# DelftMercurians/Parallax

Hardware: AMD Instinct MI355X
Metric: env steps/sec (whole node), RoboCup 4096 envs/GPU, at 1/2/4/8 MI355X (higher is better)
Workload: dtype f32

## Files before the change

__graft_entry__.py:

```python
import os
import subprocess
import sys

ROOT = os.path.dirname(os.path.abspath(__file__))
CSRC = os.path.join(ROOT, "parallax_amd", "csrc")
HIP_SRC = os.path.join(CSRC, "cotix_step.hip")
HIP_KERNEL_SRC = os.path.join(CSRC, "cotix_step_kernel.hip")
HIP_LIB = os.path.join(ROOT, "parallax_amd", "_lib", "libcotix_amd.so")
HIPCC_FLAGS = ["-O3", "--offload-arch=gfx950", "-ffp-contract=off", "-fno-fast-math", "-std=c++17", "-fPIC"]


def _run(cmd, cwd=ROOT):
    print("+", " ".join(cmd), flush=True)
    subprocess.run(cmd, cwd=cwd, check=True)


def build_id(defines=(), extra=()):
    import hashlib
    h = hashlib.sha256()
    files = sorted(f for f in os.listdir(CSRC) if f.endswith((".h", ".hip")))
    for f in files:
        h.update(f.encode())
        h.update(open(os.path.join(CSRC, f), "rb").read())
    h.update(open(os.path.join(ROOT, "include", "cotix_amd.h"), "rb").read())
# ... 10 lines not shown
    os.makedirs(os.path.dirname(out), exist_ok=True)
    hipcc = os.environ.get("HIPCC", "/opt/rocm/bin/hipcc")
    objdir = os.path.join(ROOT, "parallax_amd", "_lib", "obj", os.path.basename(out).replace(".so", ""))
    os.makedirs(objdir, exist_ok=True)
    flags = [*HIPCC_FLAGS, *["-D" + d for d in defines], *extra]
    bid = build_id(defines, extra)
    jobs = [([hipcc, *flags, '-DCOTIX_BUILD_ID="%s"' % bid, "-c", HIP_SRC,
              "-o", os.path.join(objdir, "cotix_step.o")])]
    for ew in ews:
        jobs.append([hipcc, *flags, "-DCOTIX_EW=%d" % ew, "-c", HIP_KERNEL_SRC,
                     "-o", os.path.join(objdir, "cotix_step_kernel_ew%d.o" % ew)])
    stamps = {cmd[-1]: " ".join(cmd) + "\nbuild_id " + bid for cmd in jobs}
    procs = []
    for cmd in jobs:
        if not _stale(cmd[-1], stamps[cmd[-1]]):
            continue
        print("+", " ".join(cmd), flush=True)
        procs.append((cmd, subprocess.Popen(cmd, cwd=ROOT)))
    rcs = [p.wait() for _, p in procs]
    if any(rc != 0 for rc in rcs):
        raise RuntimeError("hipcc failed (%d of %d objects)" % (sum(rc != 0 for rc in rcs), len(rcs)))
    for cmd, _ in procs:
        with open(cmd[-1] + ".cmd", "w") as f:
            f.write(stamps[cmd[-1]])
    _run([hipcc, *flags, "-shared", *[j[-1] for j in jobs], "-o", out])


def build_checkers():
    _run(["make", "-s", "-C", os.path.join(ROOT, "oracle")])
    _run(["make", "-s", "-C", os.path.join(ROOT, "tests", "emu"), "build/libcotix_emu.so"])
    _run(["make", "-s", "-C", os.path.join(ROOT, "tests", "emu"), "-f", "gradp.mk", "build/libcotix_emu_gradp.so"])
    _run(["make", "-s", "-C", os.path.join(ROOT, "tests", "emu"), "-f", "evalgrad.mk",
          "build/libcotix_emu_evalgrad.so"])


def build():
    build_hip()
    build_checkers()
    sys.path.insert(0, ROOT)
    import parallax_amd
    print("built", HIP_LIB)


def smoke():
    import numpy as np
    import torch

    sys.path.insert(0, ROOT)
    sys.path.insert(0, os.path.join(ROOT, "oracle"))
    import parallax_amd as pa
    from cotix_oracle import geometry as G
    from cotix_oracle import physics as P
    from cotix_oracle import prng

    assert torch.cuda.is_available(), "smoke() needs a GPU"
    d0 = prng.gjk_initial_direction()

    env = pa.RoboCupEnv(batch=1, device="cuda:0", keys=pa.random.PRNGKey(0, "cuda:0")[None])
    env.world.step(3, 1e-2, env.stages)
    torch.cuda.synchronize()
    got = env.world.dyn[:, :, 0].cpu().numpy()
    bodies, key = P.robocup_bodies(), prng.PRNGKey(0)
    for _ in range(3):
        bodies, key = P.robocup_step(bodies, key, d0, G.ErrorFlag())
    want = np.array([b.dyn() for b in bodies], dtype=np.float32)
    assert np.array_equal(np.isnan(got), np.isnan(want)), (got, want)
# ... 17 lines not shown
```

parallax_amd/csrc/cotix_kernel.h:

```cpp
#pragma once
#include "../../include/cotix_amd.h"
#include "cotix_device.h"
#include "cotix_grad.h"

namespace cxk {

constexpr int MAXB = 16, MAXP = 32, MAXC = 256, MAXL = 128, MAXT = 13, MAXCAND = 16384;
constexpr int MAXHOT = 24576;
constexpr int WAVE = 64;

#ifdef COTIX_STATS
struct Stats {
  unsigned long long wave_steps, active_items, rounds, resolutions, f_items, b_items, draws, valid_draws, r1_left, lvl_env, lvl_wave, e1_slots;
  unsigned long long valid_cands, fit64;
  unsigned long long bp_cand, bp_guard_fail;
  unsigned long long epa_runs;
};
inline Stats g_stats{};
#define CXK_STAT(f, v) (cxk::g_stats.f += (unsigned long long)(v))
#else
#define CXK_STAT(f, v) ((void)0)
#endif
#if defined(COTIX_PHASE_PROF) && (defined(__HIP__) || defined(__HIPCC__))
static __device__ unsigned long long g_sub_cycles[8];
#define CXK_SUB_T0 const unsigned long long cxk_sub_t0 = clock64()
#define CXK_SUB_T1(k, lane)                                                                       \
  do {                                                                                            \
    const unsigned long long dt_ = clock64() - cxk_sub_t0;                                        \
    if ((lane) == __builtin_amdgcn_readfirstlane(lane)) atomicAdd(&cxk::g_sub_cycles[k], dt_); \
  } while (0)
#else
#define CXK_SUB_T0 ((void)0)
#define CXK_SUB_T1(k, lane) ((void)0)
#endif

#define CXK_INLINE_LAMBDA __attribute__((always_inline))

#ifdef COTIX_TOOLING
#define CXK_SKIP(a, bit) (((a).dbg_skip & (bit)) != 0)
#else
#define CXK_SKIP(a, bit) false
#endif

#define CXK_HDR_FIELDS(X)                                                                                          \
  X(uint16_t, nb) X(uint16_t, np) X(uint16_t, nc) X(uint16_t, nl) X(uint16_t, nt) X(uint16_t, G) X(uint16_t, W)   \
  X(uint16_t, ncand) X(float, d0x) X(float, d0y) X(uint16_t, o_par) X(uint16_t, o_rcp) X(uint16_t, o_pbody)     \
  X(uint16_t, o_pkind) X(uint16_t, o_pn) X(uint16_t, o_pgoff) X(uint16_t, o_pwoff) X(uint16_t, o_cpa)           \
  X(uint16_t, o_cpb) X(uint16_t, o_cfn) X(uint16_t, o_ci) X(uint16_t, o_cj) X(uint16_t, o_cbeg) X(uint16_t, o_ccnt) \
  X(uint16_t, o_tn1) X(uint16_t, o_tn2) X(uint16_t, o_cand) X(uint16_t, o_cdesc) X(uint16_t, o_cmask)          \
  X(uint16_t, o_cbody) X(uint16_t, nmw) X(uint16_t, poly) X(uint16_t, rcp_all) X(uint16_t, fnset)               \
  X(uint16_t, nhot) X(uint16_t, nvt) X(uint16_t, o_vit) X(uint32_t, rcp_mask) X(uint16_t, maxv)                 \
  X(uint16_t, pminv) X(uint16_t, prng) X(uint16_t, gjk_steps) X(uint16_t, epa_cap) X(uint16_t, epa_cp)          \
  X(uint16_t, epa_body) X(float, baum) X(float, baum_dt) X(float, pc) X(uint16_t, epar)
struct SceneHdr {
// ... 1737 lines not shown
  bool any = false;
  for (int q = 0; q < sc.nmw; ++q) any |= (t.tb[sc.o_cmask + l * sc.nmw + q] & t.w(c.L.vm + q, e)) != 0u;
  return any;
}
template <int EW, bool L1 = false>
CX_DEV uint32_t m_draw(const Ctx& c, Tile<EW> t, uint32_t sw, int q, int kso, bool& pass, int kl1 = 0, int ko1 = 0) {
  using namespace cx;
  const SceneHdr& sc = c.sh;
  pass = false;
  const int base = (int)(sw & 4095u), end = (int)((sw >> 12) & 8191u), id = (int)(sw >> 25);
  const int e = id % EW, idx = base + q;
  if (idx >= end) return 0xFFFFFFFFu;
  const uint32_t cd = t.tb[sc.o_cand + idx];
  const int i1 = cd & 511u, i2 = (cd >> 9) & 511u, cid = (cd >> 18) & 511u, ty = cd >> 27;
  const float cpx = t.f(c.L.con + 4 * cid + 2, e), cpy = t.f(c.L.con + 4 * cid + 3, e);
  int ko = i2;
  if constexpr (L1) {
    ko += ty > 0 ? ko1 : 0;
    for (int p = 1; p + 1 < c.nt; ++p) ko += p < ty ? t.ti(sc.o_tn2 + p) : 0;
  }
  const key2 sk = L1 ? key2{t.w(kl1 + 2 * ko, e), t.w(kl1 + 2 * ko + 1, e)}
                     : key2{t.w(kso + 2 + 2 * ty, e), t.w(kso + 3 + 2 * ty, e)};
  const bool part = sc.prng != 0;
  const bool valid = !(isn(cpx) || isn(cpy));
  const key2 k2 = L1 ? sk : split_at_l(sk, (uint32_t)t.ti(sc.o_tn2 + ty), (uint32_t)i2, part);
  const key2 k = split_at_l(k2, (uint32_t)t.ti(sc.o_tn1 + ty), (uint32_t)i1, part);
  pass = bernoulli_l(split_at_l(k, 2u, 0u, part), sc.pc, part) & valid;
  CXK_STAT(draws, 1);
  CXK_STAT(valid_draws, valid ? 1 : 0);
  return cd;
}
struct MItem {
  int cb = 0, ce = 0, cell = 0, pos = 0, e = 0;
};
template <int EW>
CX_DEV MItem m_item(const Ctx& c, Tile<EW> t, int id) {
  const SceneHdr& sc = c.sh;
  MItem it;
  if (id < c.nl * EW) {
    const int l = id / EW;
    it.e = id % EW;
    it.cb = t.ti(sc.o_cbeg + l);
    it.ce = it.cb + t.ti(sc.o_ccnt + l);
    it.cell = c.L.m + t.ti(sc.o_ci + l) * c.nb + t.ti(sc.o_cj + l);
  }
  return it;
}
struct MConst {
  MItem it[2];
  uint32_t cm[2][2] = {{0u, 0u}, {0u, 0u}};
};
template <int EW>
CX_DEV void mc_fetch(const Ctx& c, Tile<EW> t, int lane, MConst& m) {
  const SceneHdr& sc = c.sh;
#pragma unroll
  for (int s = 0; s < 2; ++s) {
    const int id = lane + s * WAVE;
    if (s == 1 && c.nl * EW <= WAVE) continue;
    m.it[s] = m_item<EW>(c, t, id);
    if (id < c.nl * EW)
      for (int q = 0; q < 2 && q < sc.nmw; ++q) m.cm[s][q] = t.tb[sc.o_cmask + (id / EW) * sc.nmw + q];
  }
}
template <int EW>
CX_DEV bool m0_active_c(const KArgs& a, const Ctx& c, Tile<EW> t, int env0, int id, const uint32_t* cm) {
  const SceneHdr& sc = c.sh;
  if (sc.nmw > 2) return m0_active<EW>(a, c, t, env0, id);
  if (id >= c.nl * EW) return false;
  const int e = id % EW;
  if (env0 + e >= a.B) return false;
  bool any = false;
  for (int q = 0; q < 2 && q < sc.nmw; ++q) any |= (cm[q] & t.w(c.L.vm + q, e)) != 0u;
  return any;
}
template <int EW>
CX_DEV bool m_settle(Tile<EW> t, MItem& it, bool drew, uint64_t bits, uint32_t wcd, int G) {
  if (!drew) return true;
  if (bits != 0ull) {
    t.w(it.cell, it.e) = wcd;
    return false;
  }
  it.pos += G;
  return it.cb + it.pos < it.ce;
}
template <int EW, bool L1 = false>
CX_DEV void ph_M_fused(const KArgs& a, const Ctx& c, Tile<EW> t, int env0, int lane, int kso, const MConst& mc,
                       int kl1 = 0, int ko1 = 0) {
  const bool two = c.nl * EW > WAVE;
  MItem it0 = mc.it[0], it1 = mc.it[1];
  const bool f0 = m0_active_c<EW>(a, c, t, env0, lane, mc.cm[0]);
  const bool f1 = two && m0_active_c<EW>(a, c, t, env0, lane + WAVE, mc.cm[1]);
  uint64_t pend0 = ballot(f0), pend1 = two ? ballot(f1) : 0ull;
#ifdef COTIX_STATS
  {
    uint64_t nv = 0;
    for (int s = 0; s < 2; ++s) {
      const MItem& it = s ? it1 : it0;
      if (!(s ? f1 : f0)) continue;
      for (int idx = it.cb; idx < it.ce; ++idx) {
        const int cid = (t.tb[c.sh.o_cand + idx] >> 18) & 511u;
        if (!(cx::isn(t.f(c.L.con + 4 * cid + 2, it.e)) || cx::isn(t.f(c.L.con + 4 * cid + 3, it.e)))) ++nv;
      }
    }
    static uint64_t wsum = 0;
    if (lane == 0) wsum = 0;
    wsum += nv;
    if (lane == WAVE - 1) {
      CXK_STAT(valid_cands, wsum);
      CXK_STAT(fit64, wsum <= 64 ? 1 : 0);
      CXK_STAT(wave_steps, 1);
      CXK_STAT(active_items, popc64(pend0) + popc64(pend1));
    }
  }
#endif
  for (int round = 0; (pend0 | pend1) != 0ull; ++round) {
#ifdef COTIX_STATS
    if (lane == 0) {
      CXK_STAT(rounds, 1);
      if (round == 1) CXK_STAT(r1_left, popc64(pend0) + popc64(pend1));
    }
#endif
    const int n0 = popc64(pend0), n = n0 + popc64(pend1);
    const int ns = n < COTIX_SCAN_RANKS ? n : COTIX_SCAN_RANKS, G = lanes_per_item(ns);
    const bool m0 = ((pend0 >> lane) & 1ull) != 0ull, m1 = ((pend1 >> lane) & 1ull) != 0ull;
    const int r0 = popc64(pend0 & lanes_below(lane)), r1 = n0 + popc64(pend1 & lanes_below(lane));
    const bool d0 = m0 && r0 < ns, d1 = m1 && r1 < ns;
    if (d0) t.ws[WS_FLAG + r0] = (uint32_t)(it0.cb + it0.pos) | ((uint32_t)it0.ce << 12) | ((uint32_t)lane << 25);
    if (d1)
      t.ws[WS_FLAG + r1] =
          (uint32_t)(it1.cb + it1.pos) | ((uint32_t)it1.ce << 12) | ((uint32_t)(lane + WAVE) << 25);
    lockstep();
    const int slot = rank_of_lane(lane, G), q = lane - slot * G;
    bool pass = false;
    uint32_t cd = 0xFFFFFFFFu;
    if (slot < ns) cd = m_draw<EW, L1>(c, t, t.ws[WS_FLAG + slot], q, kso, pass, kl1, ko1);
    const uint64_t pm = ballot(pass);
    const uint64_t gm = G == WAVE ? ~0ull : ((1ull << G) - 1ull);
    const uint64_t b0 = d0 ? (pm >> (r0 * G)) & gm : 0ull;
    const uint32_t w0 = bpermute(b0 != 0ull ? r0 * G + __builtin_ctzll(b0) : lane, cd);
    const bool k0 = m0 && m_settle<EW>(t, it0, d0, b0, w0, G);
    pend0 = ballot(k0);
    if (two) {
      const uint64_t b1 = d1 ? (pm >> (r1 * G)) & gm : 0ull;
      const uint32_t w1 = bpermute(b1 != 0ull ? r1 * G + __builtin_ctzll(b1) : lane, cd);
      const bool k1 = m1 && m_settle<EW>(t, it1, d1, b1, w1, G);
      pend1 = ballot(k1);
    }
  }
}

CX_DEV cx::Params load_par(const uint32_t* tb, int o) {
  return cx::Params{__uint_as_float(tb[o]), __uint_as_float(tb[o + 1]), __uint_as_float(tb[o + 2]),
                    __uint_as_float(tb[o + 3])};
}
template <int EW>
CX_DEV cx::Params body_par(const Ctx& c, Tile<EW> t, int i, int e) {
  if (c.sh.epar == 0) return load_par(t.tb, c.sh.o_par + 4 * i);
  const int o = c.L.geo + (int)c.sh.epar - 1 + 4 * i;
  return cx::Params{t.f(o, e), t.f(o + 1, e), t.f(o + 2, e), t.f(o + 3, e)};
}
CX_DEV cx::Rcp load_rcp(const uint32_t* tb, int o) {
  return cx::Rcp{__uint_as_float(tb[o]), __uint_as_float(tb[o + 1])};
}

CX_HD int tape_stage(const Ctx& c) { return c.L.rec - 5 * c.nb; }
template <int EW, bool RCP>
CX_DEV void e0_item(const Ctx& c, Tile<EW> t, int e, int i, int j, int cid, bool stage = false, uint32_t* tp = nullptr) {
  using namespace cx;
  const SceneHdr& sc = c.sh;
  const Lay& L = c.L;
  const int ro = L.rp + RP_W * i;
  const bool pair = !(j == i || j < 0 || j >= c.nb) && cid >= 0;
  const int jc = pair ? j : i, co = L.con + 4 * (pair ? cid : 0);
  const v2 cp = v2{t.f(co + 2, e), t.f(co + 3, e)};
  const int oi = L.dyn + 6 * i, oj = L.dyn + 6 * jc;
  const Dyn bi = Dyn{t.f(oi, e), t.f(oi + 1, e), 0.0f, 0.0f, 0.0f, 0.0f};
  const Dyn bj = Dyn{t.f(oj, e), t.f(oj + 1, e), 0.0f, 0.0f, 0.0f, 0.0f};
  const Params pj = body_par<EW>(c, t, jc, e);
  const Rcp qj = load_rcp(t.tb, sc.o_rcp + 2 * jc);
  const ResPre p = resolve_pre<RCP>(bi, body_par<EW>(c, t, i, e), load_rcp(t.tb, sc.o_rcp + 2 * i), bj, pj, qj,
                                    v2{t.f(co, e), t.f(co + 1, e)}, cp, baum_of(sc));
// ... 1398 lines not shown
    int e = w % EW, off = w / EW, g = env0 + e;
    if (g < a.B) a.grad_dyn[(size_t)off * a.B + g] = t.f(c.L.adj + off, e);
  }
}

enum : int { PH_LOAD, PH_SAVE, PH_A, PH_T, PH_B, PH_C0, PH_C0B, PH_C1, PH_C2, PH_C3, PH_D, PH_E, PH_RET, PH_STORE,
             PH_RESTORE, PH_G, PH_ADJ, PH_F, PH_K, PH_E1, PH_R, PH_TRACE, PH_BP0, PH_BP1, PH_F0, PH_F1, PH_F2, PH_F3,
             PH_TV0, PH_TV1, PH_TV2, PH_TV3, PH_J, PH_GE, PH_COUNT };
template <int EW, int FNSET, class R>
CX_DEV void transform_phases(const KArgs& a, const Ctx& c, Tile<EW> t, int env0, const R& run) {
  {
    run(PH_T, [&](int l) { ph_T<EW, FNSET>(a, c, t, env0, l); });
    if (FNSET != FNS_ANALYTIC && c.sh.nvt > 0) {
      uint64_t redo = 0ull;
      uint32_t runs = 0u;
      run(PH_TV1, [&](int l) {
        ph_TV0<EW>(a, c, t, env0, l);
        redo = tv_redo_mask<EW>(c, t, l);
        runs = tv_chunks<EW>(c, t, redo);
        ph_TV1<EW>(a, c, t, env0, l, redo, runs);
      });
      run(PH_TV2, [&](int l) { ph_TV2<EW>(a, c, t, env0, l, redo, runs); });
      run(PH_TV3, [&](int l) { ph_TV3<EW>(a, c, t, env0, l, redo, runs); });
      if ((FNSET & FNS_CONVEX) != 0 && c.sh.poly && (a.stages & COTIX_STAGE_BROADPHASE) && !CXK_SKIP(a, 2))
        run(PH_TV3, [&](int l) { ph_TV4<EW>(a, c, t, env0, l, redo, runs); });
#ifdef COTIX_EMU_POISON
      run(PH_TV3, [&](int l) {
        for (int q = l; q < 3 * c.sh.nvt * EW; q += WAVE) t.ws[c.W.vt + q] = 0x7FBADBADu;
      });
#endif
    }
  }
}
template <int EW, int FNSET, bool PRE, class R, bool AB = false, bool TAPE = false, bool L1 = false>
CX_DEV void collider_phases(const KArgs& a, const Ctx& c, Tile<EW> t, int env0, const R& run, int slot, int kso,
                            const MConst& mc, int step = 0, int kl1 = 0, int ko1 = 0) {
  if (!AB && !CXK_SKIP(a, 1)) transform_phases<EW, FNSET>(a, c, t, env0, run);
  if ((FNSET & FNS_CONVEX) != 0 && c.sh.poly && (a.stages & COTIX_STAGE_BROADPHASE) && !CXK_SKIP(a, 2)) {
    run(PH_BP0, [&](int l) { ph_BP0<EW>(a, c, t, env0, l); });
    const int n = (int)t.ws[c.W.bl_n];
    CXK_STAT(b_items, 0);
    const bool pairs = b_pairs<FNSET>() && t.ws[c.W.bl_mode] != 0u;
    const int per_round = pairs ? WAVE / 2 : WAVE;
    for (int r = 0; r * per_round < n; ++r)
      run(PH_B, [&](int l) { ph_BP2<EW, FNSET, TAPE>(a, c, t, env0, l, r, pairs, step); });
  } else if (!AB && !CXK_SKIP(a, 2)) {
    run(PH_B, [&](int l) { ph_B<EW, FNSET, TAPE>(a, c, t, env0, l, step); });
  }
  if ((FNSET & FNS_CONVEX) != 0 && c.sh.poly && !CXK_SKIP(a, 2)) {
    for (int ch = 0; ch * WAVE < c.nc * EW; ++ch) run(PH_F0, [&](int l) { ph_F0<EW>(c, t, l, ch); });
    const int n = (int)t.ws[c.W.cf_n];
    CXK_STAT(f_items, n);
    for (int b = 0; b < n; b += CFB) {
      run(PH_F1, [&](int l) { ph_F1<EW>(c, t, l, b); });
      int TC = 0, TE = 0;
      for (int i = 0; i < CFB; ++i) {
        TC += (int)t.ws[c.W.cf_c + i];
        TE += (int)t.ws[c.W.cf_s + i] - (int)t.ws[c.W.cf_c + i];
      }
      for (int r = 0; r * WAVE < TC; ++r) run(PH_F2, [&](int l) { ph_F2<EW, false>(c, t, l, b, r); });
      for (int r = 0; r * WAVE < TE; ++r) run(PH_F2, [&](int l) { ph_F2<EW, true>(c, t, l, b, r); });
      run(PH_F3, [&](int l) { ph_F3<EW>(c, t, l, b); });
    }
  }
  if (!CXK_SKIP(a, 4) && c.nl > 0 && scan_fused<EW>(c)) {
    run(PH_C1, [&](int l) { ph_M_fused<EW, L1>(a, c, t, env0, l, kso, mc, kl1, ko1); });
  } else if (!CXK_SKIP(a, 4) && c.nl > 0) {
    for (int ch = 0; ch * WAVE < c.nl * EW; ++ch) {
      run(PH_C0, [&](int l) { ph_C0<EW>(a, c, t, env0, l, ch); });
      run(PH_C0B, [&](int l) { ph_C0b<EW>(c, t, l, ch); });
    }
    CXK_STAT(wave_steps, 1);
    CXK_STAT(active_items, t.ws[WS_N]);
    for (int par = 0; t.ws[WS_N] != 0u; par ^= 1) {
      CXK_STAT(rounds, 1);
      run(PH_C1, [&](int l) { ph_C1<EW>(a, c, t, l, par, kso); });
      run(PH_C2, [&](int l) { ph_C2<EW>(c, t, l, par); });
      run(PH_C3, [&](int l) { ph_C3<EW>(c, t, l, par); });
    }
  }
  if (!CXK_SKIP(a, 8)) run(PH_D, [&](int l) { ph_D<EW, PRE, TAPE>(a, c, t, env0, l, kso, step); });
}

template <int EW, bool ROLL, bool EVAL = false>
CX_DEV void ph_load_fwd(const KArgs& a, const Ctx& c, Tile<EW> t, int env0, int l) {
  const float r0 = (ROLL && l < EW && env0 + l < a.B) ? a.ret[env0 + l] : 0.0f;
  ph_load<EW, EVAL>(a, c, t, env0, l);
  if (ROLL) {
    for (int e = l; e < EW; e += WAVE) {
      t.f(c.L.ret, e) = 0.0f;
      t.f(c.L.nres, e) = r0;
    }
    stage_ret_terms<EW>(a, c, t, l);
  }
}
struct NoKeyHelp {
  static constexpr bool on = false;
  int kwalt = 0;
  CX_MF void bar() const {}
// ... 42 lines not shown
template <int EW>
CX_HD int help_region_words(const Ctx& c) { return (c.L.S * EW + c.W.words + EW - 1) / EW * EW; }
template <int EW>
CX_HD size_t help_lds_bytes(const SceneHdr& s, int wpb) {
  const Ctx c = make_ctx<EW>(s);
  return 4 * ((size_t)s.nhot + (size_t)wpb * (help_region_words<EW>(c) + KWIN * c.L.kww * EW));
}

constexpr int KL1R = 8;
static_assert(KWIN % KL1R == 0, "a key window is whole ring halves (key_l1_next's barrier order)");
template <class H, class = void>
struct help_l1 {
  static constexpr bool value = false;
};
template <class H>
struct help_l1<H, decltype((void)H::l1)> {
  static constexpr bool value = H::l1;
};
template <class H>
CX_MF int help_l1o(const H& h) {
  if constexpr (help_l1<H>::value)
    return h.l1o;
  else
    return 0;
}
CX_HD int key_l1_keys(const SceneHdr& s, const uint32_t* tb) {
  int n = 0;
  for (int q = 0; q < s.nt; ++q) n += (int)tb[s.o_tn2 + q];
  return n;
}
template <int EW>
CX_HD int key_l1_ring_words(int nk1) { return 2 * KL1R * 2 * nk1 * EW; }
template <int EW>
CX_HD size_t help_l1_lds_bytes(const SceneHdr& s, int wpb, int nk1) {
  return help_lds_bytes<EW>(s, wpb) + 4 * (size_t)wpb * key_l1_ring_words<EW>(nk1);
}
CX_HD int key_l1_barriers(const KArgs& a) {
  return keys_on(a) && a.n_steps > 0 ? (a.n_steps + KL1R - 1) / KL1R : 0;
}
template <int EW>
struct KeyL1 {
  KeyHelper<EW> kh;
  int l1o = 0;
  int nk1 = 0;
  int s0 = 0;
  int q = 0;
};
template <int EW>
CX_DEV void key_l1_fill(const Ctx& c, Tile<EW> tr, Tile<EW> tk, int l1o, int nk1, int s0, int n, int lane) {
  using namespace cx;
  const SceneHdr& sc = c.sh;
  const bool part = sc.prng != 0;
#ifdef COTIX_EMU_POISON
  for (int w = lane; w < KL1R * 2 * nk1 * EW; w += WAVE)
    tr.u[(l1o + (s0 % (2 * KL1R)) * 2 * nk1) * EW + w] = 0x7FBADBADu;
  lockstep();
#endif
  for (int s = s0; s < s0 + n; ++s) {
    const int ko = c.L.kw + (s % KWIN) * c.L.kww, ro = l1o + (s % (2 * KL1R)) * 2 * nk1;
    for (int w = lane; w < nk1 * EW; w += WAVE) {
      const int e = w % EW;
      int j = w / EW, ty = 0, off = 0;
      for (int p = 0; p + 1 < c.nt; ++p) {
        const int np = tk.ti(sc.o_tn2 + p);
        if (ty == p && j >= np) {
          j -= np;
          off += np;
          ty = p + 1;
        }
      }
      const uint32_t N = (uint32_t)tk.ti(sc.o_tn2 + ty);
      const key2 sk = key2{tk.w(ko + 2 + 2 * ty, e), tk.w(ko + 3 + 2 * ty, e)};
      if (part) {
        const key2 k = split_at_l(sk, N, (uint32_t)j, true);
        tr.w(ro + 2 * (off + j), e) = k.a;
        tr.w(ro + 2 * (off + j) + 1, e) = k.b;
      } else {
        const key2 r = threefry(sk, (uint32_t)j, N + (uint32_t)j);
        tr.w(ro + 2 * off + j, e) = r.a;
        tr.w(ro + 2 * off + (int)N + j, e) = r.b;
      }
    }
  }
}
template <int EW, class R>
CX_DEV void key_l1_next(const KArgs& a, const Ctx& c, KeyL1<EW>& h, const R& run) {
  KeyHelper<EW>& kh = h.kh;
  if (h.q++ == 0) {
    const int n0 = a.n_steps < KWIN ? a.n_steps : KWIN;
    run(PH_K, [&](int l) {
      const int e = l >> 1, g = kh.env0 + e;
      if (l < 2 * EW && g < a.B) kh.k = cx::key2{a.keys[2 * (size_t)g], a.keys[2 * (size_t)g + 1]};
      k0_regs<EW>(a, c, kh.th, l, n0, kh.k, true);
    });
    run(PH_K, [&](int l) { ph_K1<EW>(c, kh.th, l, n0); });
  }
  if (h.s0 > 0 && h.s0 % KWIN == 0) key_helper_next<EW>(a, c, kh, run);
  const int w = h.s0 / KWIN, n = a.n_steps - h.s0 < KL1R ? a.n_steps - h.s0 : KL1R;
  const Tile<EW> tk = (w == 0 || (w & 1)) ? kh.th : kh.tm;
  run(PH_K, [&](int l) { key_l1_fill<EW>(c, kh.tm, tk, h.l1o, h.nk1, h.s0, n, l); });
  h.s0 += KL1R;
}

template <int EW, int FNSET, bool ROLL, bool EVAL = false, bool SDEFER = false, bool ESAVE = false, class R = void,
          class H = NoKeyHelp>
CX_DEV void run_wave(const KArgs& a, const Ctx& c, Tile<EW> t, int env0, const R& run, bool loaded = false,
                     const H& help = H{}) {
  static_assert(!(ROLL && EVAL), "the rollout has no judge");
  static_assert(!ESAVE || (EVAL && !ROLL && !SDEFER), "the saving eval is the eval program");
  static_assert(!(H::on && (ROLL || EVAL)), "the key helper runs the step program only");
  constexpr bool SAVE = ROLL || ESAVE;
  uint32_t fin0 = 0u;
  if (!loaded) run(PH_LOAD, [&](int l) { ph_load_fwd<EW, ROLL, EVAL>(a, c, t, env0, l); });
  const bool keys = keys_on(a);
  constexpr bool L1 = help_l1<H>::value;
  static_assert(!L1 || H::on, "the level-1 key ring is the key helper's");
  const int nk1 = L1 ? key_l1_keys(c.sh, t.tb) : 0, ko1 = L1 && c.nt > 0 ? t.ti(c.sh.o_tn2) : 0;
  if (EVAL && a.judge.on) {
    run(PH_J, [&](int l) {
      ph_JB<EW>(a, c, t, env0, l);
      if (ESAVE) ph_jrec<EW>(a, c, t, env0, l, 0, fin0);
    });
    run(PH_J, [&](int l) { ph_JS<EW>(c, t, l); });
  }

  const bool bconst = FNSET == FNS_ANALYTIC && c.nc * EW > ABQ * WAVE && c.nc * EW <= HQ * WAVE &&
                      (a.stages & COTIX_STAGE_COLLIDER) != 0 && !CXK_SKIP(a, 2) &&
                      a.n_steps >= COTIX_BCONST_MIN_STEPS;
  BConst bc;
  if (bconst) run(PH_B, [&](int l) { bc_fetch<EW>(c, t, l, bc); });
  MConst mc;
  if ((a.stages & COTIX_STAGE_COLLIDER) && c.nl > 0 && scan_fused<EW>(c))
    run(PH_C1, [&](int l) { mc_fetch<EW>(c, t, l, mc); });
  RetRegs rr;
  if (ROLL) run(PH_RET, [&](int l) { ret_fetch<EW>(c, t, l, rr); });
  const bool awin = ROLL && act_window<EW>(a, c);
  const bool apf = ROLL ? awin : act_prefetch<EW>(a, c);
  ActRegs an, ac;
  if (!ROLL && apf) run(PH_A, [&](int l) { act_fetch<EW>(a, c, env0, l, 0, an); });
  auto act_next = [&](int l, int step) {
    if (ROLL) {
      if (awin) {
        const int o = c.L.rst + 2 * (step % AWIN);
        ac.x = t.f(o, l % EW);
        ac.y = t.f(o + 1, l % EW);
      }
    } else {
      ac = an;
      if (apf && !a.action_held && step + 1 < a.n_steps) act_fetch<EW>(a, c, env0, l, step + 1, an);
    }
  };
  const bool staged = !bconst && FNSET == FNS_ANALYTIC && c.nc * EW <= ABQ * WAVE;
  const bool defer = restart_deferred(a) && (!staged || SDEFER);
  const bool rstore = a.dyn_reset != nullptr && a.reset_mode == 1 && !(EVAL && a.judge.on);
  for (int step = 0; step < a.n_steps; ++step) {
    if (awin && step % AWIN == 0) run(PH_K, [&](int l) { act_window_fill<EW>(a, c, t, env0, l, step); });
    if (SAVE) run(PH_SAVE, [&](int l) { ph_save<EW, FNSET == FNS_ANALYTIC>(a, c, t, env0, l, step); });
    const int slot = step % KWIN;
    if (H::on && keys && slot == 0 && step > 0) {
      help.bar();
    } else if (keys && slot == 0 && !(step == 0 && k_in_prologue(a))) {
      const int n = a.n_steps - step < KWIN ? a.n_steps - step : KWIN;
      if (n == 1) {
        run(PH_K, [&](int l) {
          const uint32_t k0 = l < EW ? t.w(c.L.key, l) : 0u, k1 = l < EW ? t.w(c.L.key + 1, l) : 0u;
          k_one_regs<EW>(a, c, t, l, k0, k1);
        });
      } else {
        run(PH_K, [&](int l) { ph_K0<EW>(a, c, t, l, n); });
        run(PH_K, [&](int l) { ph_K1<EW>(c, t, l, n); });
        if (a.stages & COTIX_STAGE_COLLIDER) run(PH_K, [&](int l) { ph_K2<EW>(c, t, l, n); });
      }
    }
    const int kso = c.L.kw + (H::on && ((step / KWIN) & 1) ? help.kwalt : 0) + slot * c.L.kww;
    const int kl1 = L1 ? help_l1o(help) + (step % (2 * KL1R)) * 2 * nk1 : 0;
    const bool l1bar = L1 && keys && step % KL1R == 0 && !(slot == 0 && step > 0);
    if (bconst) {
      run(PH_A, [&](int l) {
        act_next(l, step);
        ph_A<EW, true, EVAL, true>(a, c, t, env0, l, step, slot, apf, ac);
      });
      if (a.stages & COTIX_STAGE_COLLIDER) run(PH_B, [&](int l) { ph_B_const<EW>(a, c, t, env0, l, bc); });
      if (l1bar) help.bar();
      if (a.stages & COTIX_STAGE_COLLIDER)
        collider_phases<EW, FNSET, true, R, true, SAVE, L1>(a, c, t, env0, run, slot, kso, mc, step, kl1, ko1);
    } else if (FNSET == FNS_ANALYTIC && c.nc * EW <= ABQ * WAVE) {
      run.template staged<ABRegs>(
          PH_B, [&](int l, ABRegs& r) { ab_fetch<EW, SDEFER>(a, c, t, l, r); },
          [&](int l) {
            act_next(l, step);
            ph_A<EW, true, EVAL, SDEFER>(a, c, t, env0, l, step, slot, apf, ac);
          },
          [&](int l, const ABRegs& r) { ab_contacts<EW>(a, c, t, env0, l, r); });
      if (l1bar) help.bar();
      if (a.stages & COTIX_STAGE_COLLIDER) collider_phases<EW, FNSET, true, R, FNSET == FNS_ANALYTIC, SAVE, L1>(
          a, c, t, env0, run, slot, kso, mc, step, kl1, ko1);
    } else {
      run(PH_A, [&](int l) {
        act_next(l, step);
        ph_A<EW, true, EVAL, true>(a, c, t, env0, l, step, slot, apf, ac);
      });
      if (l1bar) help.bar();
      if (a.stages & COTIX_STAGE_COLLIDER)
        collider_phases<EW, FNSET, true, R, false, SAVE, L1>(a, c, t, env0, run, slot, kso, mc, step, kl1, ko1);
    }
    if (a.trace_chosen != nullptr || a.trace_cells != nullptr)
      run(PH_TRACE, [&](int l) { ph_trace<EW>(a, c, t, env0, l, step); });
    if (!CXK_SKIP(a, 32)) {
      if (SAVE && FNSET == FNS_ANALYTIC && a.tape != nullptr && tape_rec(c.sh) && (a.stages & COTIX_STAGE_COLLIDER))
        run(PH_E1, [&](int l) { ph_E<EW, false, ROLL, true>(a, c, t, env0, l, kso, &rr); });
      else
        run(PH_E1, [&](int l) { ph_E<EW, false, ROLL>(a, c, t, env0, l, kso, &rr); });
      if (a.dyn_reset != nullptr && a.reset_mode == 1 && !defer && !(rstore && step == a.n_steps - 1))
        run(PH_R, [&](int l) { ph_R<EW>(c, t, l); });
    } else if (ROLL) {
      run(PH_RET, [&](int l) {
        for (int e = l; e < EW; e += WAVE)
          if (env0 + e < a.B) ret_accum<EW>(a, c, t, e, rr);
      });
    }
    if (EVAL && a.judge.on) {
      run(PH_J, [&](int l) {
        ph_J<EW>(a, c, t, env0, l);
        if (ESAVE) ph_jrec<EW>(a, c, t, env0, l, step + 1, fin0);
      });
      run(PH_J, [&](int l) { ph_JS<EW>(c, t, l); });
      if ((step + 1) % a.nfe_len == 0) {
        run(PH_J, [&](int l) { ph_JE<EW>(a, c, t, env0, l); });
        if (step + 1 < a.n_steps) {
          run(PH_J, [&](int l) { ph_JB<EW>(a, c, t, env0, l); });
          run(PH_J, [&](int l) { ph_JS<EW>(c, t, l); });
        }
      }
    }
  }
  if (SAVE && a.tape != nullptr && (a.stages & COTIX_STAGE_COLLIDER) && a.n_steps > 0)
    run(PH_SAVE, [&](int l) { tape_save<EW, FNSET == FNS_ANALYTIC>(a, c, t, env0, l, a.n_steps - 1); });
// ... 256 lines not shown
```

parallax_amd/csrc/cotix_plan.h:

```cpp
#pragma once
#include <algorithm>
#include <cstddef>

#include "cotix_kernel.h"

namespace cxl {
constexpr int WPB = 4;
constexpr size_t LDS_CAP = 160 * 1024;

struct StepKey {
  int fnset, mode, spec;
  bool gp;
  int ews;
};
struct HelpKey {
  int fnset, spec;
  bool sdefer, l1;
  int ews;
};
struct SplitKey {
  int nb, spec;
  int ews;
};
constexpr int F_AN = cxk::FNS_ANALYTIC, F_PP = F_AN | cxk::FNS_CONVEX, F_AP = F_PP | cxk::FNS_AABB_POLY,
// ... 102 lines not shown
  size_t lds;
  const char* error;
};
constexpr StepKey step_key(const LaunchPlan& p) { return {p.fnset, p.mode, p.spec, p.gp, 0}; }
constexpr HelpKey help_key(const LaunchPlan& p) { return {p.fnset, p.spec, p.sdefer, p.family == FAM_HELP_L1, 0}; }
constexpr SplitKey split_key(const LaunchPlan& p) { return {p.nb, p.spec, 0}; }

inline LaunchPlan plan_launch(const cxk::SceneDev& sc, int fnset, Variant v, const cxk::KArgs& a, int mode,
                              Device dev) {
  LaunchPlan p{};
  p.ew = v.envs_per_wave;
  p.wpb = scene_wpb(sc, p.ew);
  if (p.wpb == 0) {
    p.error = "scene too large for the LDS tile";
    return p;
  }
  p.fnset = cxk::launch_fnset(fnset, mode);
  p.mode = mode;
  p.nb = sc.nb;
  p.gp = a.grad_params != nullptr;
  const int spec = v.specialize && p.wpb == WPB ? cxk::spec_of(sc) : cxk::SPEC_GENERIC;
  p.spec = spec;
  p.grid = (unsigned)((a.B + WPB * 4 - 1) / (WPB * 4));
  p.block = 2 * WPB * 64;
  if (mode == 4 && dev.split_bwd_on && !p.gp && p.wpb == WPB && split_bwd_may_run(sc, fnset, p.ew, a) &&
      cxk::lds_bytes(sc, 2 * WPB, 4) <= LDS_CAP && compiled(4, split_key(p))) {
    p.family = FAM_SPLIT;
    p.lds = cxk::lds_bytes(sc, 2 * WPB, 4);
    return p;
  }
  if (mode == 0 && dev.key_helper_on && p.wpb == WPB && key_helper_may_run(fnset, p.ew, a.n_steps) &&
      cxk::help_lds_bytes<4>(sc, WPB) <= LDS_CAP) {
    const size_t lds0 = cxk::help_lds_bytes<4>(sc, WPB);
    const size_t lds1 = cxk::help_l1_lds_bytes<4>(sc, WPB, cxk::key_l1_keys(sc, sc.hot));
    const cxk::Ctx c4 = cxk::make_ctx<4>(sc);
    const int need = dev.cus > 0 ? ((int)p.grid + dev.cus - 1) / dev.cus : 2;
    const int res0 = std::min<int>(2, (int)(LDS_CAP / lds0)), res1 = std::min<int>(2, (int)(LDS_CAP / lds1));
    const bool l1 = (a.stages & COTIX_STAGE_COLLIDER) && c4.nl > 0 && cxk::scan_fused<4>(c4) && lds1 <= LDS_CAP &&
                    res1 >= std::min(res0, need);
    p.sdefer = spec == cxk::SPEC_ROBOCUP || spec == cxk::SPEC_ROBOCUP_PART;
    p.family = l1 ? FAM_HELP_L1 : FAM_HELP;
    if (compiled(4, help_key(p))) {
      p.lds = l1 ? lds1 : lds0;
      return p;
    }
    p.sdefer = false;
  }
  p.family = FAM_STEP;
  if (!compiled(p.ew, step_key(p))) p.spec = cxk::SPEC_GENERIC;
  if (!compiled(p.ew, step_key(p))) p.error = "no kernel is compiled for this launch";
  p.grid = (unsigned)((a.B + p.wpb * p.ew - 1) / (p.wpb * p.ew));
  p.block = p.wpb * 64;
  p.lds = cxk::lds_bytes(sc, p.wpb, p.ew);
  return p;
}
}
```

parallax_amd/csrc/cotix_step_kernel.hip:

```cpp
#include <hip/hip_runtime.h>

#include <array>
#include <utility>

#include "../../include/cotix_amd.h"
#include "cotix_device.h"
#include "cotix_kernel.h"
#include "cotix_launch.h"

#ifndef COTIX_EW
#error "compile with -DCOTIX_EW=1|2|4|8"
#endif

using cxk::SceneDev;

namespace {

using cxl::WPB;
#ifdef COTIX_PHASE_PROF
__device__ unsigned long long g_phase_cycles[cxk::PH_COUNT];
constexpr int STAMP_WAVES = 4096;
__device__ unsigned long long g_stamps[STAMP_WAVES * 4];
#define CXK_STAMP(v) const unsigned long long v = __builtin_amdgcn_s_memrealtime()
#else
// ... 143 lines not shown
    for (int k = 0; k < HC; ++k) {
      const int i = base + k * NT + (int)threadIdx.x;
      r[k] = i < nhot ? sc->hot[i] : 0u;
    }
#pragma unroll
    for (int k = 0; k < HC; ++k) {
      const int i = base + k * NT + (int)threadIdx.x;
      if (i < nhot) lds[i] = r[k];
    }
  }
  const cxk::Ctx c = cxk::make_ctx<EW>(sh);
  const int wave = threadIdx.x >> 6, lane = threadIdx.x & 63;
  const int grp = wave % WPB, role = wave < WPB ? 1 : 2;
  const int env0 = (blockIdx.x * WPB + grp) * EW;
  const int rw = c.L.S * EW + c.W.words;
  uint32_t* r0 = lds + nhot + grp * rw;
  uint32_t* r1 = lds + nhot + (grp + WPB) * rw;
  uint32_t* ws = (role == 1 ? r0 : r1) + c.L.S * EW;
  const cxk::Tile<EW> t0{r0, lds, ws}, t1{r1, lds, ws};
  __syncthreads();
  PhaseAcc pa;
  const WaveRun run = pa.run(lane);
  cxk::run_backward_split<EW, NB>(a, c, t0, t1, env0, run, role, [] { lds_barrier(); });
  pa.flush(lane == 0 && env0 < a.B);
}
struct GpuKeyHelp {
  static constexpr bool on = true;
  int kwalt;
  __device__ __forceinline__ void bar() const { lds_barrier(); }
};
struct GpuKeyHelpL1 {
  static constexpr bool on = true;
  static constexpr bool l1 = true;
  int kwalt;
  int l1o;
  __device__ __forceinline__ void bar() const { lds_barrier(); }
};
template <int FNSET, int SPEC, bool SDEFER, bool L1 = false>
__global__ __launch_bounds__(2 * WPB * 64) void step_help_kernel(cxk::KArgs a) {
  constexpr int EW = 4;
  extern __shared__ uint32_t lds[];
  const SceneDev* sc = a.sc;
  const cxk::SceneHdr sh = cxk::spec_hdr<SPEC>(a.sh);
  const int nhot = sh.nhot;
  constexpr int HC = 8, NT = 2 * WPB * 64;
  for (int base = 0; base < nhot; base += HC * NT) {
    uint32_t r[HC];
#pragma unroll
    for (int k = 0; k < HC; ++k) {
      const int i = base + k * NT + (int)threadIdx.x;
      r[k] = i < nhot ? sc->hot[i] : 0u;
    }
#pragma unroll
    for (int k = 0; k < HC; ++k) {
      const int i = base + k * NT + (int)threadIdx.x;
      if (i < nhot) lds[i] = r[k];
    }
  }
  const cxk::Ctx c = cxk::make_ctx<EW>(sh);
  const int wave = threadIdx.x >> 6, lane = threadIdx.x & 63;
  const int grp = wave % WPB;
  const bool stepper = wave < WPB;
  const int env0 = (blockIdx.x * WPB + grp) * EW;
  const int rw = cxk::help_region_words<EW>(c), hw = cxk::KWIN * c.L.kww * EW;
  uint32_t* um = lds + nhot + grp * rw;
  uint32_t* hb = lds + nhot + WPB * rw + grp * hw;
  const cxk::Tile<EW> tm{um, lds, um + c.L.S * EW};
  if (stepper && env0 < a.B) cxk::ph_load_fwd<EW, false>(a, c, tm, env0, lane);
  __syncthreads();
  PhaseAcc pa;
  const WaveRun run = pa.run(lane);
  const int nbar = L1 ? cxk::key_l1_barriers(a) : cxk::keys_on(a) ? cxk::key_helper_windows(a) : 0;
  if (env0 >= a.B) {
    for (int q = 0; q < nbar; ++q) lds_barrier();
    return;
  }
  if constexpr (L1) {
    const int nk1 = cxk::key_l1_keys(sh, lds);
    const int l1o = (int)(lds + nhot + WPB * (rw + hw) + grp * cxk::key_l1_ring_words<EW>(nk1) - um) / EW;
    if (stepper) {
      __builtin_amdgcn_s_setprio(2);
      const GpuKeyHelpL1 help{(int)(hb - um) / EW - c.L.kw, l1o};
      cxk::run_wave<EW, FNSET, false, false, SDEFER>(a, c, tm, env0, run, true, help);
    } else {
      cxk::KeyL1<EW> h;
      h.kh.tm = tm;
      h.kh.th = cxk::Tile<EW>{hb - c.L.kw * EW, lds, nullptr};
      h.kh.env0 = env0;
      h.l1o = l1o;
      h.nk1 = nk1;
      for (int q = 0; q < nbar; ++q) {
        cxk::key_l1_next<EW>(a, c, h, run);
        lds_barrier();
      }
    }
  } else if (stepper) {
    const GpuKeyHelp help{(int)(hb - um) / EW - c.L.kw};
    cxk::run_wave<EW, FNSET, false, false, SDEFER>(a, c, tm, env0, run, true, help);
  } else {
    cxk::KeyHelper<EW> h;
    h.tm = tm;
    h.th = cxk::Tile<EW>{hb - c.L.kw * EW, lds, nullptr};
    h.env0 = env0;
    if (nbar > 0) cxk::key_helper_init<EW>(a, c, h, run);
    for (int q = 0; q < nbar; ++q) {
      cxk::key_helper_next<EW>(a, c, h, run);
      lds_barrier();
    }
  }
  pa.flush(lane == 0 && stepper);
}
#endif

using KernelFn = void (*)(cxk::KArgs);
template <int EW, size_t I>
constexpr KernelFn step_fn() {
  constexpr cxl::StepKey k = cxl::STEP_KERNELS[I];
  if constexpr ((k.ews & EW) != 0)
    return &step_kernel<EW, k.fnset, k.mode, k.spec, k.gp>;
  else
    return nullptr;
}
template <int EW, size_t... I>
// ... 70 lines not shown
```

Measured before the change: 743.0 million.

## Speculatively precompute first scan draws in key helper wave for fused M phase

After: 781.1 million, median of 6. +5.1%, better.

```diff
diff --git a/__graft_entry__.py b/__graft_entry__.py
--- a/__graft_entry__.py
+++ b/__graft_entry__.py
@@ -66,6 +66,8 @@
     _run(["make", "-s", "-C", os.path.join(ROOT, "tests", "emu"), "-f", "gradp.mk", "build/libcotix_emu_gradp.so"])
     _run(["make", "-s", "-C", os.path.join(ROOT, "tests", "emu"), "-f", "evalgrad.mk",
           "build/libcotix_emu_evalgrad.so"])
+    _run(["make", "-s", "-C", os.path.join(ROOT, "tests", "emu"), "-f", "scanspec.mk",
+          "build/libcotix_emu_scanspec.so"])
 
 
 def build():
diff --git a/parallax_amd/csrc/cotix_kernel.h b/parallax_amd/csrc/cotix_kernel.h
--- a/parallax_amd/csrc/cotix_kernel.h
+++ b/parallax_amd/csrc/cotix_kernel.h
@@ -15,11 +15,16 @@
   unsigned long long valid_cands, fit64;
   unsigned long long bp_cand, bp_guard_fail;
   unsigned long long epa_runs;
+  unsigned long long settle[18];
 };
 inline Stats g_stats{};
+inline void (*g_settle_hook)(int lane, int at0, int len0, int at1, int len1) = nullptr;
 #define CXK_STAT(f, v) (cxk::g_stats.f += (unsigned long long)(v))
 #else
 #define CXK_STAT(f, v) ((void)0)
+#endif
+#ifdef COTIX_EMU_POISON
+inline unsigned long long g_emu_round0_done = 0;
 #endif
 #if defined(COTIX_PHASE_PROF) && (defined(__HIP__) || defined(__HIPCC__))
 static __device__ unsigned long long g_sub_cycles[8];
@@ -1823,6 +1828,9 @@
 }
 struct MItem {
   int cb = 0, ce = 0, cell = 0, pos = 0, e = 0;
+#ifdef COTIX_STATS
+  int at = -1;
+#endif
 };
 template <int EW>
 CX_DEV MItem m_item(const Ctx& c, Tile<EW> t, int id) {
@@ -1841,6 +1849,25 @@
   MItem it[2];
   uint32_t cm[2][2] = {{0u, 0u}, {0u, 0u}};
 };
+constexpr int SCAN_M_MAX = 8;
+template <int SM>
+struct MSpecIds {
+  static_assert(SM > 0 && SM <= SCAN_M_MAX && MAXC <= 256, "a byte per contact id, two words per item");
+  uint32_t w[2][(SM + 3) / 4] = {};
+};
+template <>
+struct MSpecIds<0> {};
+template <int EW, int SM>
+CX_DEV void ms_fetch(const Ctx& c, Tile<EW> t, int lane, const MConst& m, MSpecIds<SM>& ms) {
+  if constexpr (SM > 0) {
+#pragma unroll
+    for (int s = 0; s < 2; ++s) {
+      if (lane + s * WAVE >= c.nl * EW) continue;
+      for (int q = 0; q < SM && m.it[s].cb + q < m.it[s].ce; ++q)
+        ms.w[s][q >> 2] |= ((t.tb[c.sh.o_cand + m.it[s].cb + q] >> 18) & 255u) << (8 * (q & 3));
+    }
+  }
+}
 template <int EW>
 CX_DEV void mc_fetch(const Ctx& c, Tile<EW> t, int lane, MConst& m) {
   const SceneHdr& sc = c.sh;
@@ -1869,14 +1896,66 @@
   if (!drew) return true;
   if (bits != 0ull) {
     t.w(it.cell, it.e) = wcd;
+#ifdef COTIX_STATS
+    const int at = it.pos + __builtin_ctzll(bits);
+    it.at = at;
+    CXK_STAT(settle[at < 16 ? at : 16], 1);
+#endif
     return false;
   }
   it.pos += G;
+#ifdef COTIX_STATS
+  if (it.cb + it.pos >= it.ce) {
+    it.at = it.ce - it.cb;
+    CXK_STAT(settle[17], 1);
+  }
+#endif
   return it.cb + it.pos < it.ce;
 }
-template <int EW, bool L1 = false>
+template <int EW, int SM>
+CX_DEV bool m_spec(const Ctx& c, Tile<EW> t, MItem& it, int id, const uint32_t* ids, int ksp) {
+  const SceneHdr& sc = c.sh;
+  const uint32_t w = t.u[ksp * EW + id];
+  uint32_t ok = 0u;
+  if (sc.nmw <= 2) {
+    const uint64_t vv = (uint64_t)t.w(c.L.vm, it.e) | (sc.nmw > 1 ? (uint64_t)t.w(c.L.vm + 1, it.e) << 32 : 0ull);
+#pragma unroll
+    for (int m = 0; m < SM; ++m) ok |= (uint32_t)((vv >> ((ids[m >> 2] >> (8 * (m & 3))) & 255u)) & 1ull) << m;
+  } else {
+#pragma unroll
+    for (int m = 0; m < SM; ++m) {
+      const int cid = (int)((ids[m >> 2] >> (8 * (m & 3))) & 255u);
+      ok |= ((t.w(c.L.vm + (cid >> 5), it.e) >> (cid & 31)) & 1u) << m;
+    }
+  }
+  const uint32_t bits = w & ok;
+  const int len = it.ce - it.cb;
+  if (bits != 0u) {
+    t.w(it.cell, it.e) = t.tb[sc.o_cand + it.cb + __builtin_ctz(bits)];
+#ifdef COTIX_STATS
+    it.at = __builtin_ctz(bits);
+    CXK_STAT(settle[it.at], 1);
+#endif
+#ifdef COTIX_EMU_POISON
+    ++g_emu_round0_done;
+#endif
+    return false;
+  }
+  it.pos = len < SM ? len : SM;
+#ifdef COTIX_STATS
+  if (it.pos >= len) {
+    it.at = len;
+    CXK_STAT(settle[17], 1);
+  }
+#endif
+#ifdef COTIX_EMU_POISON
+  if (it.pos >= len) ++g_emu_round0_done;
+#endif
+  return it.pos < len;
+}
+template <int EW, bool L1 = false, int SM = 0>
 CX_DEV void ph_M_fused(const KArgs& a, const Ctx& c, Tile<EW> t, int env0, int lane, int kso, const MConst& mc,
-                       int kl1 = 0, int ko1 = 0) {
+                       int kl1 = 0, int ko1 = 0, int ksp = -1, const MSpecIds<SM>& ms = MSpecIds<SM>{}) {
   const bool two = c.nl * EW > WAVE;
   MItem it0 = mc.it[0], it1 = mc.it[1];
   const bool f0 = m0_active_c<EW>(a, c, t, env0, lane, mc.cm[0]);
@@ -1904,6 +1983,16 @@
     }
   }
 #endif
+  if constexpr (SM > 0) {
+    if (ksp >= 0) {
+      const bool k0 = f0 && m_spec<EW, SM>(c, t, it0, lane, ms.w[0], ksp);
+      pend0 = ballot(k0);
+      if (two) {
+        const bool k1 = f1 && m_spec<EW, SM>(c, t, it1, lane + WAVE, ms.w[1], ksp);
+        pend1 = ballot(k1);
+      }
+    }
+  }
   for (int round = 0; (pend0 | pend1) != 0ull; ++round) {
 #ifdef COTIX_STATS
     if (lane == 0) {
@@ -1938,6 +2027,10 @@
       pend1 = ballot(k1);
     }
   }
+#ifdef COTIX_STATS
+  if (g_settle_hook != nullptr)
+    g_settle_hook(lane, f0 ? it0.at : -1, it0.ce - it0.cb, f1 ? it1.at : -1, it1.ce - it1.cb);
+#endif
 }
 
 CX_DEV cx::Params load_par(const uint32_t* tb, int o) {
@@ -3402,9 +3495,10 @@
     }
   }
 }
-template <int EW, int FNSET, bool PRE, class R, bool AB = false, bool TAPE = false, bool L1 = false>
+template <int EW, int FNSET, bool PRE, class R, bool AB = false, bool TAPE = false, bool L1 = false, int SM = 0>
 CX_DEV void collider_phases(const KArgs& a, const Ctx& c, Tile<EW> t, int env0, const R& run, int slot, int kso,
-                            const MConst& mc, int step = 0, int kl1 = 0, int ko1 = 0) {
+                            const MConst& mc, int step = 0, int kl1 = 0, int ko1 = 0, int ksp = -1,
+                            const MSpecIds<SM>& ms = MSpecIds<SM>{}) {
   if (!AB && !CXK_SKIP(a, 1)) transform_phases<EW, FNSET>(a, c, t, env0, run);
   if ((FNSET & FNS_CONVEX) != 0 && c.sh.poly && (a.stages & COTIX_STAGE_BROADPHASE) && !CXK_SKIP(a, 2)) {
     run(PH_BP0, [&](int l) { ph_BP0<EW>(a, c, t, env0, l); });
@@ -3434,7 +3528,7 @@
     }
   }
   if (!CXK_SKIP(a, 4) && c.nl > 0 && scan_fused<EW>(c)) {
-    run(PH_C1, [&](int l) { ph_M_fused<EW, L1>(a, c, t, env0, l, kso, mc, kl1, ko1); });
+    run(PH_C1, [&](int l) { ph_M_fused<EW, L1, SM>(a, c, t, env0, l, kso, mc, kl1, ko1, ksp, ms); });
   } else if (!CXK_SKIP(a, 4) && c.nl > 0) {
     for (int ch = 0; ch * WAVE < c.nl * EW; ++ch) {
       run(PH_C0, [&](int l) { ph_C0<EW>(a, c, t, env0, l, ch); });
@@ -3543,11 +3637,35 @@
 template <int EW>
 CX_HD int key_l1_ring_words(int nk1) { return 2 * KL1R * 2 * nk1 * EW; }
 template <int EW>
-CX_HD size_t help_l1_lds_bytes(const SceneHdr& s, int wpb, int nk1) {
-  return help_lds_bytes<EW>(s, wpb) + 4 * (size_t)wpb * key_l1_ring_words<EW>(nk1);
+CX_HD int scan_spec_ring_words(const SceneHdr& s) { return 2 * KL1R * (int)s.nl * EW; }
+template <int EW>
+CX_HD size_t help_l1_lds_bytes(const SceneHdr& s, int wpb, int nk1, bool spec = false) {
+  return help_lds_bytes<EW>(s, wpb) +
+         4 * (size_t)wpb * (key_l1_ring_words<EW>(nk1) + (spec ? scan_spec_ring_words<EW>(s) : 0));
 }
 CX_HD int key_l1_barriers(const KArgs& a) {
   return keys_on(a) && a.n_steps > 0 ? (a.n_steps + KL1R - 1) / KL1R : 0;
+}
+#ifndef COTIX_SCAN_M
+#define COTIX_SCAN_M 4
+#endif
+constexpr int SCAN_M = COTIX_SCAN_M;
+static_assert(SCAN_M > 0 && SCAN_M <= SCAN_M_MAX && (SCAN_M & (SCAN_M - 1)) == 0 && WAVE % SCAN_M == 0,
+              "an item's draws are SCAN_M consecutive lanes of one pass");
+template <class H, class = void>
+struct help_spec {
+  static constexpr int value = 0;
+};
+template <class H>
+struct help_spec<H, decltype((void)H::spec)> {
+  static constexpr int value = H::spec;
+};
+template <class H>
+CX_MF int help_spo(const H& h) {
+  if constexpr (help_spec<H>::value > 0)
+    return h.spo;
+  else
+    return 0;
 }
 template <int EW>
 struct KeyL1 {
@@ -3556,7 +3674,39 @@
   int nk1 = 0;
   int s0 = 0;
   int q = 0;
+  int sm = 0;
+  int spo = 0;
 };
+template <int EW>
+CX_DEV void scan_spec_fill(const Ctx& c, Tile<EW> tr, int l1o, int nk1, int spo, int M, int s0, int n, int lane) {
+  using namespace cx;
+  const SceneHdr& sc = c.sh;
+  const bool part = sc.prng != 0;
+  const int NI = c.nl * EW;
+#ifdef COTIX_EMU_POISON
+  for (int w = lane; w < KL1R * NI; w += WAVE) tr.u[(spo + (s0 % (2 * KL1R)) * c.nl) * EW + w] = 0x7FBADBADu;
+  lockstep();
+#endif
+  const int total = n * NI * M;
+  for (int base = 0; base < total; base += WAVE) {
+    const int x = base + lane, m = x % M, id = (x / M) % NI, s = s0 + x / (M * NI);
+    const int l = id / EW, e = id % EW;
+    bool pass = false;
+    if (x < total && m < tr.ti(sc.o_ccnt + l)) {
+      const uint32_t cd = tr.tb[sc.o_cand + tr.ti(sc.o_cbeg + l) + m];
+      const int i1 = cd & 511u, i2 = (cd >> 9) & 511u, ty = cd >> 27;
+      int ko = i2;
+      for (int p = 0; p + 1 < c.nt; ++p) ko += p < ty ? tr.ti(sc.o_tn2 + p) : 0;
+      const int kl1 = l1o + (s % (2 * KL1R)) * 2 * nk1;
+      const key2 k2 = key2{tr.w(kl1 + 2 * ko, e), tr.w(kl1 + 2 * ko + 1, e)};
+      const key2 k = split_at_l(k2, (uint32_t)tr.ti(sc.o_tn1 + ty), (uint32_t)i1, part);
+      pass = bernoulli_l(split_at_l(k, 2u, 0u, part), sc.pc, part);
+    }
+    const uint64_t pm = ballot(pass);
+    if (x < total && m == 0)
+      tr.u[(spo + (s % (2 * KL1R)) * c.nl) * EW + id] = (uint32_t)(pm >> lane) & ((1u << M) - 1u);
+  }
+}
 template <int EW>
 CX_DEV void key_l1_fill(const Ctx& c, Tile<EW> tr, Tile<EW> tk, int l1o, int nk1, int s0, int n, int lane) {
   using namespace cx;
@@ -3610,6 +3760,8 @@
   const int w = h.s0 / KWIN, n = a.n_steps - h.s0 < KL1R ? a.n_steps - h.s0 : KL1R;
   const Tile<EW> tk = (w == 0 || (w & 1)) ? kh.th : kh.tm;
   run(PH_K, [&](int l) { key_l1_fill<EW>(c, kh.tm, tk, h.l1o, h.nk1, h.s0, n, l); });
+  if (h.sm > 0 && h.s0 > 0)
+    run(PH_K, [&](int l) { scan_spec_fill<EW>(c, kh.tm, h.l1o, h.nk1, h.spo, h.sm, h.s0, n, l); });
   h.s0 += KL1R;
 }
 
@@ -3627,6 +3779,8 @@
   constexpr bool L1 = help_l1<H>::value;
   static_assert(!L1 || H::on, "the level-1 key ring is the key helper's");
   const int nk1 = L1 ? key_l1_keys(c.sh, t.tb) : 0, ko1 = L1 && c.nt > 0 ? t.ti(c.sh.o_tn2) : 0;
+  constexpr int SM = help_spec<H>::value;
+  static_assert(SM == 0 || L1, "the speculative draws read the level-1 key ring");
   if (EVAL && a.judge.on) {
     run(PH_J, [&](int l) {
       ph_JB<EW>(a, c, t, env0, l);
@@ -3641,8 +3795,12 @@
   BConst bc;
   if (bconst) run(PH_B, [&](int l) { bc_fetch<EW>(c, t, l, bc); });
   MConst mc;
+  MSpecIds<SM> ms;
   if ((a.stages & COTIX_STAGE_COLLIDER) && c.nl > 0 && scan_fused<EW>(c))
-    run(PH_C1, [&](int l) { mc_fetch<EW>(c, t, l, mc); });
+    run(PH_C1, [&](int l) {
+      mc_fetch<EW>(c, t, l, mc);
+      ms_fetch<EW, SM>(c, t, l, mc, ms);
+    });
   RetRegs rr;
   if (ROLL) run(PH_RET, [&](int l) { ret_fetch<EW>(c, t, l, rr); });
   const bool awin = ROLL && act_window<EW>(a, c);
@@ -3686,6 +3844,7 @@
     const int kso = c.L.kw + (H::on && ((step / KWIN) & 1) ? help.kwalt : 0) + slot * c.L.kww;
     const int kl1 = L1 ? help_l1o(help) + (step % (2 * KL1R)) * 2 * nk1 : 0;
     const bool l1bar = L1 && keys && step % KL1R == 0 && !(slot == 0 && step > 0);
+    const int ksp = SM > 0 && step >= KL1R ? help_spo(help) + (step % (2 * KL1R)) * c.nl : -1;
     if (bconst) {
       run(PH_A, [&](int l) {
         act_next(l, step);
@@ -3694,7 +3853,8 @@
       if (a.stages & COTIX_STAGE_COLLIDER) run(PH_B, [&](int l) { ph_B_const<EW>(a, c, t, env0, l, bc); });
       if (l1bar) help.bar();
       if (a.stages & COTIX_STAGE_COLLIDER)
-        collider_phases<EW, FNSET, true, R, true, SAVE, L1>(a, c, t, env0, run, slot, kso, mc, step, kl1, ko1);
+        collider_phases<EW, FNSET, true, R, true, SAVE, L1, SM>(a, c, t, env0, run, slot, kso, mc, step, kl1, ko1,
+                                                                ksp, ms);
     } else if (FNSET == FNS_ANALYTIC && c.nc * EW <= ABQ * WAVE) {
       run.template staged<ABRegs>(
           PH_B, [&](int l, ABRegs& r) { ab_fetch<EW, SDEFER>(a, c, t, l, r); },
@@ -3704,8 +3864,8 @@
           },
           [&](int l, const ABRegs& r) { ab_contacts<EW>(a, c, t, env0, l, r); });
       if (l1bar) help.bar();
-      if (a.stages & COTIX_STAGE_COLLIDER) collider_phases<EW, FNSET, true, R, FNSET == FNS_ANALYTIC, SAVE, L1>(
-          a, c, t, env0, run, slot, kso, mc, step, kl1, ko1);
+      if (a.stages & COTIX_STAGE_COLLIDER) collider_phases<EW, FNSET, true, R, FNSET == FNS_ANALYTIC, SAVE, L1, SM>(
+          a, c, t, env0, run, slot, kso, mc, step, kl1, ko1, ksp, ms);
     } else {
       run(PH_A, [&](int l) {
         act_next(l, step);
@@ -3713,7 +3873,8 @@
       });
       if (l1bar) help.bar();
       if (a.stages & COTIX_STAGE_COLLIDER)
-        collider_phases<EW, FNSET, true, R, false, SAVE, L1>(a, c, t, env0, run, slot, kso, mc, step, kl1, ko1);
+        collider_phases<EW, FNSET, true, R, false, SAVE, L1, SM>(a, c, t, env0, run, slot, kso, mc, step, kl1, ko1,
+                                                                 ksp, ms);
     }
     if (a.trace_chosen != nullptr || a.trace_cells != nullptr)
       run(PH_TRACE, [&](int l) { ph_trace<EW>(a, c, t, env0, l, step); });
diff --git a/parallax_amd/csrc/cotix_plan.h b/parallax_amd/csrc/cotix_plan.h
--- a/parallax_amd/csrc/cotix_plan.h
+++ b/parallax_amd/csrc/cotix_plan.h
@@ -158,7 +158,7 @@
   if (mode == 0 && dev.key_helper_on && p.wpb == WPB && key_helper_may_run(fnset, p.ew, a.n_steps) &&
       cxk::help_lds_bytes<4>(sc, WPB) <= LDS_CAP) {
     const size_t lds0 = cxk::help_lds_bytes<4>(sc, WPB);
-    const size_t lds1 = cxk::help_l1_lds_bytes<4>(sc, WPB, cxk::key_l1_keys(sc, sc.hot));
+    const size_t lds1 = cxk::help_l1_lds_bytes<4>(sc, WPB, cxk::key_l1_keys(sc, sc.hot), true);
     const cxk::Ctx c4 = cxk::make_ctx<4>(sc);
     const int need = dev.cus > 0 ? ((int)p.grid + dev.cus - 1) / dev.cus : 2;
     const int res0 = std::min<int>(2, (int)(LDS_CAP / lds0)), res1 = std::min<int>(2, (int)(LDS_CAP / lds1));
diff --git a/parallax_amd/csrc/cotix_step_kernel.hip b/parallax_amd/csrc/cotix_step_kernel.hip
--- a/parallax_amd/csrc/cotix_step_kernel.hip
+++ b/parallax_amd/csrc/cotix_step_kernel.hip
@@ -199,8 +199,10 @@
 struct GpuKeyHelpL1 {
   static constexpr bool on = true;
   static constexpr bool l1 = true;
+  static constexpr int spec = cxk::SCAN_M;
   int kwalt;
   int l1o;
+  int spo;
   __device__ __forceinline__ void bar() const { lds_barrier(); }
 };
 template <int FNSET, int SPEC, bool SDEFER, bool L1 = false>
@@ -245,9 +247,11 @@
   if constexpr (L1) {
     const int nk1 = cxk::key_l1_keys(sh, lds);
     const int l1o = (int)(lds + nhot + WPB * (rw + hw) + grp * cxk::key_l1_ring_words<EW>(nk1) - um) / EW;
+    const int spo = (int)(lds + nhot + WPB * (rw + hw + cxk::key_l1_ring_words<EW>(nk1)) +
+                          grp * cxk::scan_spec_ring_words<EW>(sh) - um) / EW;
     if (stepper) {
       __builtin_amdgcn_s_setprio(2);
-      const GpuKeyHelpL1 help{(int)(hb - um) / EW - c.L.kw, l1o};
+      const GpuKeyHelpL1 help{(int)(hb - um) / EW - c.L.kw, l1o, spo};
       cxk::run_wave<EW, FNSET, false, false, SDEFER>(a, c, tm, env0, run, true, help);
     } else {
       cxk::KeyL1<EW> h;
@@ -256,6 +260,8 @@
       h.kh.env0 = env0;
       h.l1o = l1o;
       h.nk1 = nk1;
+      h.sm = cxk::SCAN_M;
+      h.spo = spo;
       for (int q = 0; q < nbar; ++q) {
         cxk::key_l1_next<EW>(a, c, h, run);
         lds_barrier();
```
